# YzM1a0/MuDPT

Hardware: AMD Instinct MI355X
Metric: images/sec fwd+bwd ViT-B/16 MuDPT (higher is better)
Workload: dtype bf16; 1 GPU; MuDPT ViT-B/16 fwd+bwd+SGD, batch 256/GPU, 11 class prompts, n_ctx 4, depth 12, synthetic 224x224 N(0,1) images, random-init frozen CLIP (BASELINE configs[1]); global_batch=256, parallelism=dp1

## Files before the change

mudpt_amd/csrc/gemm.hip:

```cpp
#include <type_traits>

#include "kernels.h"

namespace mudpt {

using gptr_t = const __attribute__((address_space(1))) void*;
using lptr_t = __attribute__((address_space(3))) void*;

template <typename T, int BM, int BN, int WM, int WN, int EPI, int NS = 2, int BK = 64>
__global__ __launch_bounds__(WM* WN * 64) void gemm_nt_kernel(GemmArgs p) {
    using elem = typename T::elem;
    using vec8 = typename T::vec8;
    constexpr int NW = WM * WN;
    static_assert(BK == 64 || BK == 128, "K-tile");
    constexpr int ROWB = BK * 2;
    constexpr int RPI = 1024 / ROWB;
    constexpr int CPR = ROWB / 16;
    constexpr int TM = BM / WM / 16;
    constexpr int TN = BN / WN / 16;
    constexpr int IA = BM / RPI / NW;
    constexpr int IB = BN / RPI / NW;
    constexpr int STAGE_BYTES = (BM + BN) * ROWB;
    static_assert(BM % (RPI * NW) == 0 && BN % (RPI * NW) == 0, "tile rows must split over the waves");

    extern __shared__ __attribute__((aligned(16))) char smem[];

    const int tid = threadIdx.x;
    const int lane = tid & 63;
    const int wave = __builtin_amdgcn_readfirstlane(tid >> 6);
    const int wm = wave / WN, wn = wave % WN;

    const int ntn = (p.N + BN - 1) / BN;
    const int wg = (p.flags & 1) ? (int)blockIdx.x : xcd_remap(blockIdx.x, gridDim.x);
    const int m0 = (wg / ntn) * BM;
    const int n0 = (wg % ntn) * BN;

    const int kz = blockIdx.y, kspan = p.ksplit ? p.ksplit : p.K;
    const elem* __restrict__ A = (const elem*)p.A + (size_t)kz * kspan;
    const elem* __restrict__ Bw = (const elem*)p.B + (size_t)kz * kspan;

    const int srow = lane / CPR;
    const elem* asrc[IA];
    const elem* bsrc[IB];
#pragma unroll
    for (int i = 0; i < IA; ++i) {
        const int tr = (wave + NW * i) * RPI + srow;
        int r = m0 + tr;
        r = r < p.M ? r : p.M - 1;
        asrc[i] = A + (size_t)r * p.lda + ((lane % CPR) ^ (tr & (CPR - 1))) * 8;
    }
#pragma unroll
    for (int i = 0; i < IB; ++i) {
        const int tr = (wave + NW * i) * RPI + srow;
        int r = n0 + tr;
        r = r < p.N ? r : p.N - 1;
        bsrc[i] = Bw + (size_t)r * p.ldb + ((lane % CPR) ^ (tr & (CPR - 1))) * 8;
    }

    const int nt1 = kspan / BK;
    const bool f8 = p.lo_mode == LO_F8;
    const int nt = nt1 + (p.lo_mode == LO_NONE ? 0 : (f8 ? nt1 / 2 : nt1));
    const ptrdiff_t dA = p.A_lo ? (const char*)p.A_lo - (const char*)p.A : 0;
    const ptrdiff_t dB = f8 ? (const char*)p.B8 - (const char*)p.B : 0;
    auto stage = [&](int buf, int kt) {
        char* base = smem + buf * STAGE_BYTES;
        const bool second = kt >= nt1;
        const ptrdiff_t oa = second ? dA + (ptrdiff_t)(kt - nt1) * ROWB : (ptrdiff_t)kt * ROWB;
        const ptrdiff_t ob = second ? dB + (ptrdiff_t)(kt - nt1) * ROWB : (ptrdiff_t)kt * ROWB;
#pragma unroll
        for (int i = 0; i < IA; ++i)
            __builtin_amdgcn_global_load_lds((gptr_t)((const char*)asrc[i] + oa), (lptr_t)(base + (wave + NW * i) * 1024), 16, 0, 0);
#pragma unroll
        for (int i = 0; i < IB; ++i)
            __builtin_amdgcn_global_load_lds((gptr_t)((const char*)bsrc[i] + ob), (lptr_t)(base + BM * ROWB + (wave + NW * i) * 1024), 16, 0, 0);
    };

    f32x4 acc[TM][TN];
#pragma unroll
    for (int i = 0; i < TM; ++i)
#pragma unroll
        for (int j = 0; j < TN; ++j) acc[i][j] = f32x4{0.f, 0.f, 0.f, 0.f};

    const int frow = lane & 15;
    const int fq = lane >> 4;
    int aoff[TM], boff[TN];
#pragma unroll
    for (int i = 0; i < TM; ++i) aoff[i] = (wm * (BM / WM) + i * 16 + frow) * ROWB;
#pragma unroll
    for (int j = 0; j < TN; ++j) boff[j] = BM * ROWB + (wn * (BN / WN) + j * 16 + frow) * ROWB;
    const int sw = frow & (CPR - 1);

    static_assert(NS >= 2 && (NS & (NS - 1)) == 0, "ring depth must be a power of two");
#pragma unroll
    for (int st = 0; st < NS - 1; ++st)
        if (st < nt) stage(st, st);

    auto tile = [&](auto f8tag, int kt) {
        const int cur = kt & (NS - 1);
        if (kt + NS - 2 < nt) asm volatile("s_waitcnt vmcnt(%0)" ::"n"((NS - 2) * (IA + IB)) : "memory");
        else asm volatile("s_waitcnt vmcnt(0)" ::: "memory");
        __syncthreads();
        if (kt + NS - 1 < nt) stage((kt + NS - 1) & (NS - 1), kt + NS - 1);
        const char* base = smem + cur * STAGE_BYTES;
        if constexpr (decltype(f8tag)::value && BK == 64) {
            const int c = ((2 * fq) ^ sw) * 16;
            typedef __attribute__((ext_vector_type(4))) int i32x4;
            i32x8 b8[TN];
#pragma unroll
            for (int j = 0; j < TN; ++j)
                b8[j] = __builtin_shufflevector(*(const i32x4*)(base + boff[j] + c), *(const i32x4*)(base + boff[j] + (c ^ 16)), 0, 1, 2, 3, 4, 5, 6, 7);
#pragma unroll
            for (int i = 0; i < TM; ++i) {
                const i32x8 a8 = __builtin_shufflevector(*(const i32x4*)(base + aoff[i] + c), *(const i32x4*)(base + aoff[i] + (c ^ 16)), 0, 1, 2, 3, 4, 5, 6, 7);
#pragma unroll
                for (int j = 0; j < TN; ++j)
                    acc[i][j] = __builtin_amdgcn_mfma_scale_f32_16x16x128_f8f6f4(b8[j], a8, acc[i][j], 0, 0, 0, p.b8_scale, 0, LO8_SCALE_E8M0);
            }
        } else {
#pragma unroll
            for (int ks = 0; ks < BK / 32; ++ks) {
                const int c = ((ks * 4 + fq) ^ sw) * 16;
                vec8 af[TM], bf[TN];
#pragma unroll
                for (int i = 0; i < TM; ++i) af[i] = *(const vec8*)(base + aoff[i] + c);
#pragma unroll
                for (int j = 0; j < TN; ++j) bf[j] = *(const vec8*)(base + boff[j] + c);
#pragma unroll
                for (int i = 0; i < TM; ++i)
#pragma unroll
                    for (int j = 0; j < TN; ++j) acc[i][j] = T::mfma16(bf[j], af[i], acc[i][j]);
            }
        }
    };
    const int nt16 = f8 ? nt1 : nt;
    for (int kt = 0; kt < nt16; ++kt) tile(std::false_type{}, kt);
    for (int kt = nt16; kt < nt; ++kt) tile(std::true_type{}, kt);

#pragma unroll
    for (int i = 0; i < TM; ++i) {
        const int m = m0 + wm * (BM / WM) + i * 16 + frow;
        if (m >= p.M) continue;
        size_t orow = (size_t)m;
        const float* posrow = nullptr;
        if constexpr (EPI == EPI_PATCH) {
            const int b = m / p.patches, pp = m - b * p.patches;
            orow = (size_t)b * p.seq_len + 1 + pp;
            posrow = p.pos + (size_t)(1 + pp) * p.N;
        }
#pragma unroll
        for (int j = 0; j < TN; ++j) {
            const int n = n0 + wn * (BN / WN) + j * 16 + fq * 4;
            if (n >= p.N) continue;
            f32x4 v = acc[i][j];
            if (p.bias) {
                const f32x4 b4 = *(const f32x4*)(p.bias + n);
                v += b4;
            }
            if constexpr (EPI == EPI_STORE) {
                typename T::vec4 o = {round_to<elem>(v[0]), round_to<elem>(v[1]), round_to<elem>(v[2]), round_to<elem>(v[3])};
                *(typename T::vec4*)((elem*)p.out0 + orow * p.ldo0 + n) = o;
            } else if constexpr (EPI == EPI_GELU) {
                if (p.gelu_q8) {
                    *(uint32_t*)((char*)p.out0 + orow * p.ldo0 + n) = gelu_grad_q8x4(v[0], v[1], v[2], v[3]);
                } else {
                    typename T::vec4 u = {round_to<elem>(v[0]), round_to<elem>(v[1]), round_to<elem>(v[2]), round_to<elem>(v[3])};
                    *(typename T::vec4*)((elem*)p.out0 + orow * p.ldo0 + n) = u;
                }
                if (p.out1_lo) {
                    typename T::vec4 g, lo;
                    float rem[4];
#pragma unroll
                    for (int c = 0; c < 4; ++c) { elem hv; rem[c] = split_rem(quick_gelu(v[c]), hv); g[c] = hv; lo[c] = (elem)rem[c]; }
                    *(typename T::vec4*)((elem*)p.out1 + orow * p.ldo1 + n) = g;
                    if (p.out1_lo_mode == LO_F8) *(uint32_t*)((char*)p.out1_lo + orow * p.ldo1 * 2 + n) = pack_lo8(rem[0], rem[1], rem[2], rem[3]);
                    else *(typename T::vec4*)((elem*)p.out1_lo + orow * p.ldo1 + n) = lo;
                } else {
                    typename T::vec4 g = {round_to<elem>(quick_gelu(v[0])), round_to<elem>(quick_gelu(v[1])), round_to<elem>(quick_gelu(v[2])), round_to<elem>(quick_gelu(v[3]))};
                    *(typename T::vec4*)((elem*)p.out1 + orow * p.ldo1 + n) = g;
                }
            } else if constexpr (EPI == EPI_RESIDUAL) {
                const f32x4 r4 = *(const f32x4*)((const float*)p.aux + orow * p.ldaux + n);
                *(f32x4*)((float*)p.out0 + orow * p.ldo0 + n) = v + r4;
            } else if constexpr (EPI == EPI_GELU_BWD) {
                typename T::vec4 o;
                if (p.gelu_q8) {
                    const uint32_t w = *(const uint32_t*)((const char*)p.aux + orow * p.ldaux + n);
#pragma unroll
                    for (int c = 0; c < 4; ++c) o[c] = round_to<elem>(v[c] * gelu_grad_from_q8(w, c));
                } else {
                    const typename T::vec4 u = *(const typename T::vec4*)((const elem*)p.aux + orow * p.ldaux + n);
#pragma unroll
                    for (int c = 0; c < 4; ++c) o[c] = round_to<elem>(v[c] * quick_gelu_grad((float)u[c]));
                }
                *(typename T::vec4*)((elem*)p.out0 + orow * p.ldo0 + n) = o;
            } else if constexpr (EPI == EPI_PATCH) {
                const f32x4 q4 = *(const f32x4*)(posrow + n);
                *(f32x4*)((float*)p.out0 + orow * p.ldo0 + n) = v + q4;
            } else {
                *(f32x4*)((float*)p.out0 + (size_t)kz * p.split_stride + orow * p.ldo0 + n) = v;
            }
        }
    }
}

template <typename T, int BM, int BN, int WM, int WN, int EPI, int NS = 2, int BK = 64>
static int launch_cfg(const GemmArgs& a, hipStream_t s) {
    constexpr int lds = NS * (BM + BN) * BK * 2;
    constexpr auto kern = gemm_nt_kernel<T, BM, BN, WM, WN, EPI, NS, BK>;
    if (int e = lds_limit_once<kern>(current_device(), lds)) return e;
    const int ntm = (a.M + BM - 1) / BM, ntn = (a.N + BN - 1) / BN;
    hipLaunchKernelGGL(kern, dim3(ntm * ntn, a.ksplit ? a.K / a.ksplit : 1), dim3(WM * WN * 64), lds, s, a);
    HIP_TRY(hipGetLastError());
    return MUDPT_OK;
}

static inline bool small_tiles(const GemmArgs& a) {
    const size_t t64 = (size_t)((a.M + 63) / 64) * ((a.N + 63) / 64);
    return t64 <= 1280 || (t64 <= 2560 && a.K <= 512);
}

int device_cus(int dev) {
    static int ncu[64] = {};
    if (ncu[dev] <= 0) {
        const hipError_t e = hipDeviceGetAttribute(&ncu[dev], hipDeviceAttributeMultiprocessorCount, dev);
        if (e != hipSuccess) {
            set_error("%s:%d: hipDeviceGetAttribute(MultiprocessorCount, device %d) -> %s", __FILE__, __LINE__, dev, hipGetErrorString(e));
            return ncu[dev] = 0;
        }
    }
    return ncu[dev];
}
static int cus_or_256() {
    const int n = device_cus(current_device());
    return n > 0 ? n : 256;
}

static inline bool deep_k_tiles(const GemmArgs& a, int slices, int variant, int ncu) {
    const size_t t64 = (size_t)((a.M + 63) / 64) * ((a.N + 63) / 64);
    return (variant & 0xff) != 12 && a.lo_mode == LO_NONE && (a.K / slices) % 128 == 0 && t64 * slices <= (size_t)2 * ncu;
}

static GemmForm tile_form(const GemmArgs& a, int variant, int ncu) {
    if ((size_t)a.M * a.N >= (size_t)256 * 128 * 512) {
        switch (variant & 0xff) {
            case 2: return GEMM_T128x256;
            case 4: return GEMM_T256x128;
            default: return GEMM_T256x256;
        }
    }
    const size_t t128 = (size_t)((a.M + 127) / 128) * ((a.N + 127) / 128);
    const int v = variant & 0xff;
    if (((v == 0 && small_tiles(a)) || v == 10) && deep_k_tiles(a, 1, variant, ncu)) return GEMM_T64x64_K128;
    if (((v == 0 || v == 12) && small_tiles(a)) || v == 9 || v == 10) return GEMM_T64x64;
    if ((t128 <= 128 && v != 5) || v == 6) return GEMM_T128x64_RING4;
    return GEMM_T128x128;
}

template <typename T, int EPI>
static int launch_epi(GemmForm f, const GemmArgs& a, hipStream_t s) {
    switch (f) {
        case GEMM_T256x256: return launch_cfg<T, 256, 256, 2, 4, EPI>(a, s);
        case GEMM_T128x256: return launch_cfg<T, 128, 256, 2, 4, EPI>(a, s);
        case GEMM_T256x128: return launch_cfg<T, 256, 128, 4, 2, EPI>(a, s);
        case GEMM_T64x64_K128: return launch_cfg<T, 64, 64, 2, 2, EPI, 2, 128>(a, s);
        case GEMM_T64x64: return launch_cfg<T, 64, 64, 2, 2, EPI, 2>(a, s);
        case GEMM_T128x64_RING4: return launch_cfg<T, 128, 64, 2, 2, EPI, 4>(a, s);
        case GEMM_T128x128: return launch_cfg<T, 128, 128, 2, 2, EPI>(a, s);
        default: break;
    }
    set_error("gemm: form %d is not a simple tile", (int)f);
    return MUDPT_ERR_ARG;
}

template <typename T>
static int launch_t(int epi, GemmForm f, const GemmArgs& a, hipStream_t s) {
    switch (epi) {
        case EPI_STORE: return launch_epi<T, EPI_STORE>(f, a, s);
        case EPI_GELU: return launch_epi<T, EPI_GELU>(f, a, s);
        case EPI_RESIDUAL: return launch_epi<T, EPI_RESIDUAL>(f, a, s);
        case EPI_GELU_BWD: return launch_epi<T, EPI_GELU_BWD>(f, a, s);
        case EPI_PATCH: return launch_epi<T, EPI_PATCH>(f, a, s);
        case EPI_STORE_F32: return launch_epi<T, EPI_STORE_F32>(f, a, s);
    }
    set_error("gemm: unknown epilogue %d", epi);
    return MUDPT_ERR_ARG;
}

template <typename T, bool OUT_F32>
__global__ __launch_bounds__(256) void splitk_reduce_kernel(const float* __restrict__ part, int S, size_t stride, int M, int N, const float* __restrict__ bias,
                                                            void* __restrict__ out, int ldo) {
    const size_t i = (size_t)blockIdx.x * 256 + threadIdx.x, n4 = (size_t)N / 4;
    if (i >= (size_t)M * n4) return;
    const size_t m = i / n4, n = (i - m * n4) * 4;
    f32x4 v = *(const f32x4*)(part + m * N + n);
    for (int z = 1; z < S; ++z) v += *(const f32x4*)(part + (size_t)z * stride + m * N + n);
    if (bias) v += *(const f32x4*)(bias + n);
    if constexpr (OUT_F32) {
        *(f32x4*)((float*)out + m * ldo + n) = v;
    } else {
        using elem = typename T::elem;
        typename T::vec4 o = {round_to<elem>(v[0]), round_to<elem>(v[1]), round_to<elem>(v[2]), round_to<elem>(v[3])};
        *(typename T::vec4*)((elem*)out + m * ldo + n) = o;
    }
}

static int split_k_slices(int epi, const GemmArgs& a, const GemmOpts& o, int ncu, bool& deep) {
    deep = false;
    const int v = o.variant & 0xff;
    if (!(epi == EPI_STORE || epi == EPI_STORE_F32) || !o.scratch || (v != 0 && v != 12) || a.lo_mode != LO_NONE) return 1;
    const size_t tiles = (size_t)((a.M + 63) / 64) * ((a.N + 63) / 64);
    if (tiles * 2 > (size_t)ncu * 5 || a.K < 1536) return 1;
    int S = (int)((size_t)ncu * 2 / tiles);
    if (S > 4) S = 4;
    while (S > 1 && (a.K % (S * 128) != 0 || a.K / S < 512)) --S;
    if (S >= 3 && deep_k_tiles(a, S, o.variant, ncu) && (size_t)S * a.M * a.N <= o.scratch_elems) { deep = true; return S; }
    S = (int)((size_t)ncu * 5 / tiles);
    if (S > 4) S = 4;
    while (S > 1 && (a.K % (S * 64) != 0 || a.K / S < 512)) --S;
    if ((size_t)S * a.M * a.N > o.scratch_elems) return 1;
    return S;
}

bool gemm_uses_pp(int epi, const GemmArgs& a, int variant) {
    const bool pp_epi = epi == EPI_STORE || epi == EPI_GELU || epi == EPI_GELU_BWD || epi == EPI_STORE_F32;
    const int v = variant & 0xff;
    const size_t tiles = (size_t)((a.M + 255) / 256) * ((a.N + 255) / 256);
    return (v == 0 || v == 3 || v == 5 || v == 6 || v == 12) && pp_epi && tiles >= (v == 3 ? 256 : 128) && a.ldo0 % 8 == 0 && (epi != EPI_GELU || a.ldo1 % 8 == 0) &&
           (epi != EPI_GELU_BWD || a.ldaux % 8 == 0);
}

GemmPlan gemm_form(int epi, const GemmArgs& a, const GemmOpts& o, int ncu) {
    if (gemm_uses_pp(epi, a, o.variant)) return {GEMM_PP, 1};
    bool deep = false;
    if (const int S = split_k_slices(epi, a, o, ncu, deep); S > 1) return {deep ? GEMM_SPLITK_K128 : GEMM_SPLITK_K64, S};
    return {tile_form(a, o.variant, ncu), 1};
}

bool gemm_shape_ok(int epi, const GemmArgs& a) {
    if (epi < EPI_STORE || epi > EPI_STORE_F32) return false;
    if (!(a.M > 0 && a.N > 0 && a.K > 0) || a.K % 64 != 0 || a.N % 16 != 0) return false;
    if (!(a.ldo0 >= a.N && a.ldo0 % 4 == 0)) return false;
    if (epi == EPI_GELU && !(a.ldo1 >= a.N && a.ldo1 % 4 == 0)) return false;
    if ((epi == EPI_RESIDUAL || epi == EPI_GELU_BWD) && !(a.ldaux >= a.N && a.ldaux % 4 == 0)) return false;
    if (!(a.lo_mode == LO_NONE || a.lo_mode == LO_F16 || a.lo_mode == LO_F8)) return false;
    return a.lo_mode != LO_F8 || a.K % 128 == 0;
}

int launch_gemm(int dtype, int epi, const GemmArgs& a, hipStream_t s, const GemmOpts& o) {
    const int variant = o.variant;
    ARG_CHECK(a.A && a.B && a.out0, "gemm: null operand");
    ARG_CHECK(a.M > 0 && a.N > 0 && a.K > 0, "gemm: empty shape M=%d N=%d K=%d", a.M, a.N, a.K);
    ARG_CHECK(a.K % 64 == 0, "gemm: K=%d must be a multiple of 64", a.K);
    ARG_CHECK(a.N % 16 == 0, "gemm: N=%d must be a multiple of 16", a.N);
    ARG_CHECK(a.lda >= a.K && a.ldb >= a.K && a.lda % 8 == 0 && a.ldb % 8 == 0, "gemm: bad lda/ldb %d/%d", a.lda, a.ldb);
    ARG_CHECK(a.ldo0 >= a.N && a.ldo0 % 4 == 0, "gemm: bad ldo0 %d", a.ldo0);
    ARG_CHECK(((uintptr_t)a.A % 16 == 0) && ((uintptr_t)a.B % 16 == 0) && ((uintptr_t)a.out0 % 16 == 0), "gemm: operands must be 16-byte aligned");
    if (epi == EPI_GELU) ARG_CHECK(a.out1 && a.ldo1 >= a.N && a.ldo1 % 4 == 0, "gemm: gelu epilogue needs out1");
    ARG_CHECK(!a.out1_lo || a.out1_lo_mode == LO_F16 || a.out1_lo_mode == LO_F8, "gemm: bad out1_lo_mode %d", a.out1_lo_mode);
    ARG_CHECK(!a.gelu_q8 || ((epi == EPI_GELU && !a.out1_lo) || epi == EPI_GELU_BWD), "gemm: gelu_q8 belongs to the QuickGELU epilogues (1 without a split output, 3)");
    ARG_CHECK(a.lo_mode == LO_NONE || a.lo_mode == LO_F16 || a.lo_mode == LO_F8, "gemm: bad lo_mode %d", a.lo_mode);
    if (a.lo_mode != LO_NONE) ARG_CHECK(a.A_lo && (uintptr_t)a.A_lo % 16 == 0, "gemm: a split operand needs its low half (16-byte aligned)");
    if (a.lo_mode == LO_F8) {
        ARG_CHECK(dtype == DT_F16, "gemm: the e4m3 second pass exists for fp16 operands only");
        ARG_CHECK(a.B8 && (uintptr_t)a.B8 % 16 == 0 && a.K % 128 == 0, "gemm: the e4m3 second pass needs B8 and K %% 128 == 0 (K = %d)", a.K);
        ARG_CHECK(a.b8_scale > 0 && a.b8_scale < 255, "gemm: bad E8M0 weight scale %d", a.b8_scale);
    }
    if (epi == EPI_RESIDUAL || epi == EPI_GELU_BWD) ARG_CHECK(a.aux && a.ldaux >= a.N && a.ldaux % 4 == 0, "gemm: epilogue needs aux");
    if (epi == EPI_PATCH) ARG_CHECK(a.pos && a.patches > 0 && a.seq_len > a.patches && a.M % a.patches == 0, "gemm: bad patch epilogue args");
    GemmArgs b = a;
    if (variant & 0x100) b.flags |= 1;
    if (variant & 0x200) b.flags |= 2;
    b.flags |= ((variant >> 10) & 3) << 4;
    b.flags |= ((variant >> 12) & 0xff) << 8;
    const GemmPlan plan = gemm_form(epi, a, o, cus_or_256());
    if (plan.form == GEMM_PP) return launch_gemm_pp(dtype, epi, b, s, o);
    if (plan.slices > 1) {
        const int S = plan.slices;
        const bool deep = plan.form == GEMM_SPLITK_K128;
        GemmArgs q = b;
        q.bias = nullptr; q.out0 = o.scratch; q.ldo0 = a.N; q.ksplit = a.K / S; q.split_stride = (size_t)a.M * a.N;
        if (dtype == DT_BF16) { if (int rc = deep ? launch_cfg<BF16, 64, 64, 2, 2, EPI_STORE_F32, 2, 128>(q, s) : launch_cfg<BF16, 64, 64, 2, 2, EPI_STORE_F32, 2>(q, s)) return rc; }
        else if (dtype == DT_F16) { if (int rc = deep ? launch_cfg<F16, 64, 64, 2, 2, EPI_STORE_F32, 2, 128>(q, s) : launch_cfg<F16, 64, 64, 2, 2, EPI_STORE_F32, 2>(q, s)) return rc; }
        else { set_error("gemm: unknown dtype %d", dtype); return MUDPT_ERR_ARG; }
        const unsigned grid = (unsigned)(((size_t)a.M * (a.N / 4) + 255) / 256);
        if (epi == EPI_STORE_F32) hipLaunchKernelGGL((splitk_reduce_kernel<BF16, true>), dim3(grid), dim3(256), 0, s, o.scratch, S, q.split_stride, a.M, a.N, a.bias, a.out0, a.ldo0);
        else if (dtype == DT_BF16) hipLaunchKernelGGL((splitk_reduce_kernel<BF16, false>), dim3(grid), dim3(256), 0, s, o.scratch, S, q.split_stride, a.M, a.N, a.bias, a.out0, a.ldo0);
        else hipLaunchKernelGGL((splitk_reduce_kernel<F16, false>), dim3(grid), dim3(256), 0, s, o.scratch, S, q.split_stride, a.M, a.N, a.bias, a.out0, a.ldo0);
        HIP_TRY(hipGetLastError());
        return MUDPT_OK;
    }
    if (dtype == DT_BF16) return launch_t<BF16>(epi, plan.form, b, s);
    if (dtype == DT_F16) return launch_t<F16>(epi, plan.form, b, s);
    set_error("gemm: unknown dtype %d", dtype);
    return MUDPT_ERR_ARG;
}

}
```

mudpt_amd/csrc/gemm_pp.hip:

```cpp
#include <hip/hip_ext.h>

#include <type_traits>

#include "kernels.h"

namespace mudpt {

using lptr_t = __attribute__((address_space(3))) void*;

#define VMCNT(n) asm volatile("s_waitcnt vmcnt(" #n ")" ::: "memory")
typedef __attribute__((ext_vector_type(4))) unsigned int u32x4;

template <int N>
__device__ inline void vmcnt() {
    static_assert(N >= 0 && N <= 63, "vmcnt immediate is 6 bits");
    asm volatile("s_waitcnt vmcnt(%0)" ::"n"(N) : "memory");
}

constexpr int EPI_GELU_SPLIT = 100;
constexpr int EPI_GELU_SPLIT8 = 101;
constexpr int EPI_GELU_Q8 = 102;
constexpr int EPI_GELU_BWD_Q8 = 103;

template <typename T, int EPI, bool F8 = false, int ST = 0, int LD = 0, int ABL = 0>
__global__ __launch_bounds__(512) void gemm_pp_kernel(GemmArgs p, int ntn, int ntiles, int rem_half) {
    using elem = typename T::elem;
    using vec8 = typename T::vec8;
    constexpr int STAGE = 65536, BOFF = 32768;
    extern __shared__ __attribute__((aligned(16))) char smem[];

    const int tid = threadIdx.x, lane = tid & 63;
    const int w = __builtin_amdgcn_readfirstlane(tid >> 6);
    const int wr = w >> 2, wc = w & 3;
    const int frow = lane & 15, fq = lane >> 4;

    const int nkt1 = p.K >> 6;
    const int nkt = nkt1 + (p.lo_mode == LO_NONE ? 0 : (F8 ? nkt1 >> 1 : nkt1));
    const int G = gridDim.x;
    const int my_full = rem_half ? ntiles / G : (ntiles - (int)blockIdx.x + G - 1) / G;
    const bool has_half = rem_half && (int)blockIdx.x < 2 * rem_half;
    const int total = (my_full + (has_half ? 1 : 0)) * nkt;

    const auto rsA = __builtin_amdgcn_make_buffer_rsrc(const_cast<void*>(p.A), 0, (int)((size_t)p.M * p.lda * 2 < 0xffffffffull ? (size_t)p.M * p.lda * 2 : 0xffffffffull), 0x00020000);
    const auto rsB = __builtin_amdgcn_make_buffer_rsrc(const_cast<void*>(p.B), 0, (int)((size_t)p.N * p.ldb * 2 < 0xffffffffull ? (size_t)p.N * p.ldb * 2 : 0xffffffffull), 0x00020000);
    const auto rsA2 = __builtin_amdgcn_make_buffer_rsrc(const_cast<void*>(p.A_lo ? p.A_lo : p.A), 0, (int)((size_t)p.M * p.lda * 2 < 0xffffffffull ? (size_t)p.M * p.lda * 2 : 0xffffffffull), 0x00020000);
    const auto rsB2 = __builtin_amdgcn_make_buffer_rsrc(const_cast<void*>(F8 ? p.B8 : p.B), 0, (int)((size_t)p.N * p.ldb * 2 < 0xffffffffull ? (size_t)p.N * p.ldb * 2 : 0xffffffffull), 0x00020000);

    static_assert(EPI == EPI_STORE || EPI == EPI_GELU || EPI == EPI_GELU_SPLIT || EPI == EPI_GELU_SPLIT8 || EPI == EPI_GELU_BWD || EPI == EPI_STORE_F32 ||
                  EPI == EPI_GELU_Q8 || EPI == EPI_GELU_BWD_Q8, "epilogue not built for gemm_pp");
    constexpr bool GELU = (EPI == EPI_GELU || EPI == EPI_GELU_SPLIT || EPI == EPI_GELU_SPLIT8 || EPI == EPI_GELU_Q8);
    constexpr int OOB = (int)0x80000000;
    constexpr bool OUT_F32 = (EPI == EPI_STORE_F32);
    constexpr bool NAT = OUT_F32;
    constexpr int NST = (EPI == EPI_STORE || EPI == EPI_GELU_BWD || EPI == EPI_GELU_BWD_Q8) ? 16 : (EPI == EPI_GELU_SPLIT ? 48 : (EPI == EPI_GELU_SPLIT8 ? 40 : (EPI == EPI_GELU_Q8 ? 24 : 32)));
    const auto rsOut0 = __builtin_amdgcn_make_buffer_rsrc(p.out0, 0, p.M * p.ldo0 * (OUT_F32 ? 4 : (EPI == EPI_GELU_Q8 ? 1 : 2)), 0x00020000);
    const auto rsOut1 = __builtin_amdgcn_make_buffer_rsrc(p.out1, 0, GELU ? p.M * p.ldo1 * 2 : 0, 0x00020000);
    const auto rsOut1Lo = __builtin_amdgcn_make_buffer_rsrc(p.out1_lo, 0, (EPI == EPI_GELU_SPLIT || EPI == EPI_GELU_SPLIT8) ? p.M * p.ldo1 * 2 : 0, 0x00020000);
    const auto rsAux = __builtin_amdgcn_make_buffer_rsrc(const_cast<void*>(p.aux), 0, EPI == EPI_GELU_BWD ? p.M * p.ldaux * 2 : (EPI == EPI_GELU_BWD_Q8 ? p.M * p.ldaux : 0), 0x00020000);
    const auto rsBias = __builtin_amdgcn_make_buffer_rsrc(const_cast<float*>(p.bias), 0, p.bias ? p.N * 4 : 0, 0x00020000);
    bool epi_pending = false;

    int grp[4][2];
#pragma unroll
    for (int q = 0; q < 2; ++q) {
        const int k = 2 * w + q;
        grp[0][q] = k < 8 ? k : k + 8;
        grp[3][q] = k < 8 ? k + 8 : k + 16;
        grp[1][q] = NAT ? (k >> 2) * 8 + (k & 3) : 2 * k;
        grp[2][q] = NAT ? (k >> 2) * 8 + (k & 3) + 4 : 2 * k + 1;
    }
    const int srow = lane >> 3, sslot = lane & 7;
    int lane_off[4][2];
#pragma unroll
    for (int u = 0; u < 4; ++u)
#pragma unroll
        for (int q = 0; q < 2; ++q) {
            const bool isA = (u == 0 || u == 3);
            const int row = grp[u][q] * 8 + srow;
            const int f = (isA || NAT) ? (row & 7) : ((row & 3) | (((row >> 4) & 1) << 2));
            lane_off[u][q] = (row * (isA ? p.lda : p.ldb) + ((sslot ^ f) << 3)) * 2;
        }

    const int gn_knob = (p.flags >> 8) & 0xff;
    const int GN = gn_knob > 0 ? gn_knob : (ntn >= 12 ? 6 : (ntn >= 6 && ntn % 3 == 0 ? 3 : ntn));
    const int ntm = ntiles / ntn;
    auto tile_mn = [&](int tile, int& tm, int& tn) {
        const int tpg = ntm * GN, full = ntn / GN, ng = tile / tpg;
        if (ng < full) {
            const int rem = tile - ng * tpg;
            tm = rem / GN;
            tn = ng * GN + (rem - tm * GN);
        } else {
            const int wl = ntn - full * GN, rem = tile - full * tpg;
            tm = rem / wl;
            tn = full * GN + (rem - tm * wl);
        }
    };
    auto item_tile = [&](int it, int& tm, int& tn, int& h) {
        if (it < my_full) {
            tile_mn(xcd_remap((int)blockIdx.x + it * G, ntiles), tm, tn);
            h = 0;
        } else {
            h = (int)blockIdx.x >= rem_half ? 1 : 0;
            tile_mn(xcd_remap(my_full * G + (int)blockIdx.x - h * rem_half, ntiles), tm, tn);
        }
    };
    int n_kt = 0, n_it = 0, n_baseA = 0, n_baseB = 0, n_soff = 0;
    bool n_second = false;
    bool n_half = false;
    auto set_next_item = [&](int it) {
        int tm, tn, h;
        item_tile(it, tm, tn, h);
        n_half = it >= my_full;
        n_baseA = (tm * 256 + (n_half ? h * 128 - (w >= 4 ? 64 : 0) : 0)) * p.lda * 2;
        n_baseB = tn * 256 * p.ldb * 2;
    };
    auto advance_next = [&]() {
        n_soff += 128;
        if (++n_kt == nkt) {
            n_kt = 0; n_soff = 0; n_second = false;
            if ((++n_it) * nkt < total) set_next_item(n_it);
        } else if (n_kt == nkt1) {
            n_soff = 0; n_second = true;
        }
    };
    auto issue = [&](int u, int stage) {
        if constexpr (ABL & 2) return;
        const bool isA = (u == 0 || u == 3);
        const int base = isA ? n_baseA : n_baseB;
        char* dst = smem + stage * STAGE + (isA ? 0 : BOFF);
#pragma unroll
        for (int q = 0; q < 2; ++q)
            __builtin_amdgcn_raw_ptr_buffer_load_lds(isA ? (n_second ? rsA2 : rsA) : (n_second ? rsB2 : rsB), (lptr_t)(dst + grp[u][q] * 1024), 16, lane_off[u][q] + base, n_soff, 0, 0);
    };

    const int sw = frow & 7;
    const int c0 = (fq ^ sw) << 4;
    const int c8 = ((2 * fq) ^ sw) << 4;
    int ca = c0, cb = c0 ^ 64;
    const int a_base = (wr * 128 + frow) * 128;
    const int b_base = BOFF + (NAT ? wc * 64 + frow : wc * 64 + (frow >> 2) * 16 + (frow & 3)) * 128;
    constexpr int BJ = NAT ? 2048 : 512;

    f32x4 acc[8][4];
#pragma unroll
    for (int i = 0; i < 8; ++i)
#pragma unroll
        for (int j = 0; j < 4; ++j) acc[i][j] = f32x4{0.f, 0.f, 0.f, 0.f};

    if (total > 0) {
        set_next_item(0);
        issue(0, 0); issue(1, 0); issue(2, 0);
        if (!n_half) issue(3, 0);
        advance_next();
    }
    VMCNT(0);
    __builtin_amdgcn_s_barrier();
    if (wr == 1) __builtin_amdgcn_s_barrier();

    typedef __attribute__((ext_vector_type(4))) int i32x4;
    i32x8 af[4], bf[4];
    if constexpr (ABL & 1) {
#pragma unroll
        for (int i = 0; i < 4; ++i) { af[i] = i32x8{lane, 1, 2, 3, 4, 5, 6, 7} * 0x3c003c00; bf[i] = i32x8{7, 6, 5, 4, 3, 2, 1, lane} * 0x3c003c00; }
    }
    auto half = [](const i32x8& v, int ks) -> vec8 {
        return __builtin_bit_cast(vec8, ks ? __builtin_shufflevector(v, v, 4, 5, 6, 7) : __builtin_shufflevector(v, v, 0, 1, 2, 3));
    };
    int c_it = 0;

    auto mfma_quadrant = [&](auto f8tag, int i0, int j0) {
        __builtin_amdgcn_sched_barrier(0);
        __builtin_amdgcn_s_setprio(1);
        if constexpr (decltype(f8tag)::value) {
#pragma unroll
            for (int i = 0; i < 4; ++i)
#pragma unroll
                for (int j = 0; j < 2; ++j)
                    acc[i0 + i][j0 + j] = __builtin_amdgcn_mfma_scale_f32_16x16x128_f8f6f4(bf[j0 + j], af[i], acc[i0 + i][j0 + j], 0, 0, 0, p.b8_scale, 0, LO8_SCALE_E8M0);
        } else {
#pragma unroll
            for (int ks = 0; ks < 2; ++ks)
#pragma unroll
                for (int i = 0; i < 4; ++i)
#pragma unroll
                    for (int j = 0; j < 2; ++j) acc[i0 + i][j0 + j] = T::mfma16(half(bf[j0 + j], ks), half(af[i], ks), acc[i0 + i][j0 + j]);
        }
        __builtin_amdgcn_s_setprio(0);
        __builtin_amdgcn_sched_barrier(0);
    };
    auto read_a = [&](const char* st, int i0) {
        if constexpr (ABL & 1) return;
#pragma unroll
        for (int i = 0; i < 4; ++i)
            af[i] = __builtin_shufflevector(*(const i32x4*)(st + a_base + (i0 + i) * 2048 + ca), *(const i32x4*)(st + a_base + (i0 + i) * 2048 + cb), 0, 1, 2, 3, 4, 5, 6, 7);
    };
    auto read_b = [&](const char* st, int j0) {
        if constexpr (ABL & 1) return;
#pragma unroll
        for (int j = j0; j < j0 + 2; ++j)
            bf[j] = __builtin_shufflevector(*(const i32x4*)(st + b_base + j * BJ + ca), *(const i32x4*)(st + b_base + j * BJ + cb), 0, 1, 2, 3, 4, 5, 6, 7);
    };
    auto epilogue = [&]() {
            int tm, tn, h;
            const bool c_half = c_it >= my_full;
            item_tile(c_it++, tm, tn, h);
            const int ni = c_half ? 4 : 8;
            const int n = tn * 256 + wc * 64 + (NAT ? fq * 4 : fq * 16);
            f32x4 bias4[4];
#pragma unroll
            for (int j = 0; j < 4; ++j)
                bias4[j] = p.bias ? __builtin_bit_cast(f32x4, __builtin_amdgcn_raw_buffer_load_b128(rsBias, (n + (NAT ? 16 : 4) * j) * 4, 0, 0)) : f32x4{0.f, 0.f, 0.f, 0.f};
            const int m_base = tm * 256 + (c_half ? h * 128 + wr * 64 : wr * 128) + frow;
            auto row_off = [&](int i, int ld, int esz, int col) { return (col < p.N ? (m_base * ld + col) * esz : OOB) + i * (16 * ld * esz); };
#pragma unroll
            for (int i = 0; i < 8; ++i)
#pragma unroll
                for (int j = 0; j < 4; ++j) acc[i][j] += bias4[j];
            if constexpr (EPI == EPI_GELU_BWD) {
                vec8 u[8][2];
#pragma unroll
                for (int i = 0; i < 8; ++i) {
                    const int off = i < ni ? row_off(i, p.ldaux, 2, n) : OOB;
                    u[i][0] = __builtin_bit_cast(vec8, __builtin_amdgcn_raw_buffer_load_b128(rsAux, off, 0, LD));
                    u[i][1] = __builtin_bit_cast(vec8, __builtin_amdgcn_raw_buffer_load_b128(rsAux, off, 16, LD));
                }
#pragma unroll
                for (int i = 0; i < 8; ++i)
#pragma unroll
                    for (int j = 0; j < 4; ++j)
#pragma unroll
                        for (int c = 0; c < 4; ++c) acc[i][j][c] *= quick_gelu_grad((float)u[i][j >> 1][4 * (j & 1) + c]);
            }
            if constexpr (EPI == EPI_GELU_BWD_Q8) {
                u32x4 q[8];
#pragma unroll
                for (int i = 0; i < 8; ++i) q[i] = __builtin_amdgcn_raw_buffer_load_b128(rsAux, i < ni ? row_off(i, p.ldaux, 1, n) : OOB, 0, LD);
#pragma unroll
                for (int i = 0; i < 8; ++i)
#pragma unroll
                    for (int j = 0; j < 4; ++j)
#pragma unroll
                        for (int c = 0; c < 4; ++c) acc[i][j][c] *= gelu_grad_from_q8(q[i][j], c);
            }
            __builtin_amdgcn_sched_barrier(0);
#pragma unroll
            for (int i = 0; i < 8; ++i) {
                if (i < ni) {
                if constexpr (OUT_F32) {
#pragma unroll
                    for (int j = 0; j < 4; ++j) __builtin_amdgcn_raw_buffer_store_b128(__builtin_bit_cast(u32x4, acc[i][j]), rsOut0, row_off(i, p.ldo0, 4, n + 16 * j), 0, ST);
                } else {
                    vec8 o0, o1;
                    if constexpr (EPI == EPI_GELU_Q8) {
                        u32x4 q;
#pragma unroll
                        for (int j = 0; j < 4; ++j) q[j] = gelu_grad_q8x4(acc[i][j][0], acc[i][j][1], acc[i][j][2], acc[i][j][3]);
                        __builtin_amdgcn_raw_buffer_store_b128(q, rsOut0, row_off(i, p.ldo0, 1, n), 0, ST);
                    } else {
#pragma unroll
                        for (int c = 0; c < 4; ++c) {
                            o0[c] = round_to<elem>(acc[i][0][c]); o0[4 + c] = round_to<elem>(acc[i][1][c]);
                            o1[c] = round_to<elem>(acc[i][2][c]); o1[4 + c] = round_to<elem>(acc[i][3][c]);
                        }
                        const int off = row_off(i, p.ldo0, 2, n);
                        __builtin_amdgcn_raw_buffer_store_b128(__builtin_bit_cast(u32x4, o0), rsOut0, off, 0, ST);
                        __builtin_amdgcn_raw_buffer_store_b128(__builtin_bit_cast(u32x4, o1), rsOut0, off, 16, ST);
                    }
                    if constexpr (EPI == EPI_GELU || EPI == EPI_GELU_Q8) {
#pragma unroll
                        for (int c = 0; c < 4; ++c) {
                            o0[c] = round_to<elem>(quick_gelu(acc[i][0][c])); o0[4 + c] = round_to<elem>(quick_gelu(acc[i][1][c]));
                            o1[c] = round_to<elem>(quick_gelu(acc[i][2][c])); o1[4 + c] = round_to<elem>(quick_gelu(acc[i][3][c]));
                        }
                        const int off1 = row_off(i, p.ldo1, 2, n);
                        __builtin_amdgcn_raw_buffer_store_b128(__builtin_bit_cast(u32x4, o0), rsOut1, off1, 0, ST);
                        __builtin_amdgcn_raw_buffer_store_b128(__builtin_bit_cast(u32x4, o1), rsOut1, off1, 16, ST);
                    }
                    if constexpr (EPI == EPI_GELU_SPLIT8) {
                        u32x4 l8;
                        float rem[4];
#pragma unroll
                        for (int j = 0; j < 4; ++j) {
#pragma unroll
                            for (int c = 0; c < 4; ++c) {
                                elem hv;
                                rem[c] = split_rem(quick_gelu(acc[i][j][c]), hv);
                                if (j < 2) o0[4 * j + c] = hv; else o1[4 * (j - 2) + c] = hv;
                            }
                            l8[j] = pack_lo8(rem[0], rem[1], rem[2], rem[3]);
                        }
                        const int off1 = row_off(i, p.ldo1, 2, n);
                        __builtin_amdgcn_raw_buffer_store_b128(__builtin_bit_cast(u32x4, o0), rsOut1, off1, 0, ST);
                        __builtin_amdgcn_raw_buffer_store_b128(__builtin_bit_cast(u32x4, o1), rsOut1, off1, 16, ST);
                        __builtin_amdgcn_raw_buffer_store_b128(l8, rsOut1Lo, (n < p.N ? m_base * p.ldo1 * 2 + n : OOB) + i * (32 * p.ldo1), 0, ST);
                    }
                    if constexpr (EPI == EPI_GELU_SPLIT) {
                        vec8 l0, l1;
#pragma unroll
                        for (int c = 0; c < 4; ++c) {
                            elem hv, lv;
                            split_hi_lo(quick_gelu(acc[i][0][c]), hv, lv); o0[c] = hv; l0[c] = lv;
                            split_hi_lo(quick_gelu(acc[i][1][c]), hv, lv); o0[4 + c] = hv; l0[4 + c] = lv;
                            split_hi_lo(quick_gelu(acc[i][2][c]), hv, lv); o1[c] = hv; l1[c] = lv;
                            split_hi_lo(quick_gelu(acc[i][3][c]), hv, lv); o1[4 + c] = hv; l1[4 + c] = lv;
                        }
                        const int off1 = row_off(i, p.ldo1, 2, n);
                        __builtin_amdgcn_raw_buffer_store_b128(__builtin_bit_cast(u32x4, o0), rsOut1, off1, 0, ST);
                        __builtin_amdgcn_raw_buffer_store_b128(__builtin_bit_cast(u32x4, o1), rsOut1, off1, 16, ST);
                        __builtin_amdgcn_raw_buffer_store_b128(__builtin_bit_cast(u32x4, l0), rsOut1Lo, off1, 0, ST);
                        __builtin_amdgcn_raw_buffer_store_b128(__builtin_bit_cast(u32x4, l1), rsOut1Lo, off1, 16, ST);
                    }
                }
                }
#pragma unroll
                for (int j = 0; j < 4; ++j) acc[i][j] = f32x4{0.f, 0.f, 0.f, 0.f};
            }
            epi_pending = true;
    };

    int s = 0;
    auto full_step = [&](auto f8tag) {
        constexpr bool F8S = decltype(f8tag)::value;
        const int cur = s & 1;
        const char* st = smem + cur * STAGE;
        const bool nxt = s + 1 < total;
        ca = F8S ? c8 : c0;
        cb = F8S ? (c8 ^ 16) : (c0 ^ 64);
        read_a(st, 0);
        read_b(st, 0);
        if (nxt) {
            issue(0, cur ^ 1);
            if (epi_pending) vmcnt<NST + 4>(); else vmcnt<4>();
        } else {
            if (epi_pending) vmcnt<NST + 2>(); else vmcnt<2>();
        }
        __builtin_amdgcn_s_barrier();
        mfma_quadrant(f8tag, 0, 0);
        __builtin_amdgcn_s_barrier();
        read_b(st, 2);
        if (nxt) {
            issue(1, cur ^ 1);
            if (epi_pending) vmcnt<NST + 4>(); else vmcnt<4>();
        } else {
            if (epi_pending) vmcnt<NST>(); else vmcnt<0>();
        }
        epi_pending = false;
        __builtin_amdgcn_s_barrier();
        mfma_quadrant(f8tag, 0, 2);
        __builtin_amdgcn_s_barrier();
        read_a(st, 4);
        if (nxt) issue(2, cur ^ 1);
        __builtin_amdgcn_s_barrier();
        mfma_quadrant(f8tag, 4, 2);
        __builtin_amdgcn_s_barrier();
        if (nxt) {
            if (!n_half) { issue(3, cur ^ 1); advance_next(); VMCNT(4); } else { advance_next(); VMCNT(2); }
        }
        __builtin_amdgcn_s_barrier();
        mfma_quadrant(f8tag, 4, 0);
        __builtin_amdgcn_s_barrier();
        ++s;
    };
    auto half_step = [&](auto f8tag) {
        constexpr bool F8S = decltype(f8tag)::value;
        const int cur = s & 1;
        const char* st = smem + cur * STAGE;
        const bool nxt = s + 1 < total;
        ca = F8S ? c8 : c0;
        cb = F8S ? (c8 ^ 16) : (c0 ^ 64);
        read_a(st, 0);
        read_b(st, 0);
        if (nxt) {
            issue(0, cur ^ 1);
            issue(1, cur ^ 1);
            if (epi_pending) vmcnt<NST + 4>(); else vmcnt<4>();
        } else {
            if (epi_pending) vmcnt<NST>(); else vmcnt<0>();
        }
        __builtin_amdgcn_s_barrier();
        mfma_quadrant(f8tag, 0, 0);
        __builtin_amdgcn_s_barrier();
        read_b(st, 2);
        if (nxt) { issue(2, cur ^ 1); advance_next(); VMCNT(2); }
        epi_pending = false;
        __builtin_amdgcn_s_barrier();
        mfma_quadrant(f8tag, 0, 2);
        __builtin_amdgcn_s_barrier();
        ++s;
    };
    const int nkt2 = nkt - nkt1;
    for (int it = 0; it < my_full; ++it) {
        if constexpr (F8) {
            for (int k = 0; k < nkt1; ++k) full_step(std::false_type{});
            for (int k = 0; k < nkt2; ++k) full_step(std::true_type{});
        } else {
            for (int k = 0; k < nkt; ++k) full_step(std::false_type{});
        }
        epilogue();
    }
    if (has_half) {
        if constexpr (F8) {
            for (int k = 0; k < nkt1; ++k) half_step(std::false_type{});
            for (int k = 0; k < nkt2; ++k) half_step(std::true_type{});
        } else {
            for (int k = 0; k < nkt; ++k) half_step(std::false_type{});
        }
        epilogue();
    }
    if (wr == 0) __builtin_amdgcn_s_barrier();
}

template <typename T, int EPI, bool F8 = false, int ST = 0, int LD = 0, int ABL = 0>
static int launch_pp(const GemmArgs& a, hipStream_t s, const GemmOpts& o) {
    constexpr int lds = 2 * 65536;
    constexpr auto kern = gemm_pp_kernel<T, EPI, F8, ST, LD, ABL>;
    const int dev = current_device(), ncu = device_cus(dev);
    if (ncu <= 0) return MUDPT_ERR_HIP;
    if (int e = lds_limit_once<kern>(dev, lds)) return e;
    const int ntm = (a.M + 255) / 256, ntn = (a.N + 255) / 256, ntiles = ntm * ntn;
    int grid = ntiles < ncu ? (2 * ntiles <= ncu ? 2 * ntiles : ntiles) : ncu;
    if (a.flags & 2) grid = ntiles < ncu ? ntiles : ncu;
    const int rem = ntiles % grid, rem_half = (rem > 0 && 2 * rem <= grid && !(a.flags & 2)) ? rem : 0;
    if (o.ev_start && o.ev_stop) {
        hipExtLaunchKernelGGL(kern, dim3(grid), dim3(512), lds, s, o.ev_start, o.ev_stop, 0, a, ntn, ntiles, rem_half);
    } else {
        hipLaunchKernelGGL(kern, dim3(grid), dim3(512), lds, s, a, ntn, ntiles, rem_half);
    }
    HIP_TRY(hipGetLastError());
    return MUDPT_OK;
}

template <typename T>
static int launch_pp_t(int epi, const GemmArgs& a, hipStream_t s, const GemmOpts& o) {
    if constexpr (T::id == DT_F16) {
        if (a.lo_mode == LO_F8) {
            switch (epi) {
                case EPI_STORE: return launch_pp<T, EPI_STORE, true>(a, s, o);
                case EPI_GELU:
                    if (!a.out1_lo) return launch_pp<T, EPI_GELU, true>(a, s, o);
                    return a.out1_lo_mode == LO_F8 ? launch_pp<T, EPI_GELU_SPLIT8, true>(a, s, o) : launch_pp<T, EPI_GELU_SPLIT, true>(a, s, o);
                case EPI_STORE_F32: return launch_pp<T, EPI_STORE_F32, true>(a, s, o);
            }
            set_error("gemm_pp: epilogue %d is not built with the e4m3 second pass", epi);
            return MUDPT_ERR_ARG;
        }
    }
    if constexpr (T::id == DT_BF16) {
        if (epi == EPI_STORE && (a.flags & 0x30)) {
            switch ((a.flags >> 4) & 3) {
                case 1: return launch_pp<T, EPI_STORE, false, 0, 0, 1>(a, s, o);
                case 2: return launch_pp<T, EPI_STORE, false, 0, 0, 2>(a, s, o);
                default: return launch_pp<T, EPI_STORE, false, 0, 0, 3>(a, s, o);
            }
        }
    }
    switch (epi) {
        case EPI_STORE: return launch_pp<T, EPI_STORE>(a, s, o);
        case EPI_GELU:
            if (!a.out1_lo) return a.gelu_q8 ? launch_pp<T, EPI_GELU_Q8>(a, s, o) : launch_pp<T, EPI_GELU>(a, s, o);
            return a.out1_lo_mode == LO_F8 ? launch_pp<T, EPI_GELU_SPLIT8>(a, s, o) : launch_pp<T, EPI_GELU_SPLIT>(a, s, o);
        case EPI_GELU_BWD: return a.gelu_q8 ? launch_pp<T, EPI_GELU_BWD_Q8>(a, s, o) : launch_pp<T, EPI_GELU_BWD>(a, s, o);
        case EPI_STORE_F32: return launch_pp<T, EPI_STORE_F32>(a, s, o);
    }
    set_error("gemm_pp: epilogue %d is not built for the ping-pong kernel", epi);
    return MUDPT_ERR_ARG;
}

int launch_gemm_pp(int dtype, int epi, const GemmArgs& a, hipStream_t s, const GemmOpts& o) {
    ARG_CHECK((size_t)a.M * a.lda * 2 < 0xffffffffull && (size_t)a.N * a.ldb * 2 < 0xffffffffull, "gemm_pp: operand larger than 4 GiB");
    ARG_CHECK(a.lda % 8 == 0 && a.ldb % 8 == 0 && a.ldo0 % 8 == 0, "gemm_pp: strides must be multiples of 8");
    ARG_CHECK(!a.out1_lo || (uintptr_t)a.out1_lo % 16 == 0, "gemm_pp: out1_lo must be 16-byte aligned");
    ARG_CHECK(!a.gelu_q8 || (a.lo_mode == LO_NONE && a.ldo0 % 16 == 0 && a.ldaux % 16 == 0), "gemm_pp: gelu_q8 needs 16-byte row strides and no split operand");
    ARG_CHECK((size_t)a.M * a.ldo0 * (epi == EPI_STORE_F32 ? 4 : 2) < 0x7fffffffull && (size_t)a.M * (size_t)(a.ldo1 > a.ldaux ? a.ldo1 : a.ldaux) * 2 < 0x7fffffffull, "gemm_pp: output larger than 2 GiB");
    if (dtype == DT_BF16) return launch_pp_t<BF16>(epi, a, s, o);
    if (dtype == DT_F16) return launch_pp_t<F16>(epi, a, s, o);
    set_error("gemm: unknown dtype %d", dtype);
    return MUDPT_ERR_ARG;
}

}
```

Measured before the change: 10870 images/s.

## Remap ping-pong GEMM B-fragment layout for dense epilogue stores, add cache-policy variants

Changes how B rows are assigned to LDS groups and which output columns each lane owns, so dense epilogues (store, GELU, GELU-bwd, q8) write two split column chunks per row instead of one contiguous 32-byte span. The q8 paths move from 128-bit to 64-bit loads and stores, and the stride check is relaxed to match. It also adds a variant bit field that selects nontemporal store or load cache policies per output for bf16 kernels. This affects the default store pattern of every dense ping-pong GEMM and could change coalescing either way.

Result: no change. 10840 images/s (-0.2%).

```diff
diff --git a/mudpt_amd/csrc/gemm.hip b/mudpt_amd/csrc/gemm.hip
--- a/mudpt_amd/csrc/gemm.hip
+++ b/mudpt_amd/csrc/gemm.hip
@@ -372,6 +372,7 @@
     if (variant & 0x200) b.flags |= 2;
     b.flags |= ((variant >> 10) & 3) << 4;
     b.flags |= ((variant >> 12) & 0xff) << 8;
+    b.flags |= ((variant >> 20) & 3) << 16;
     const GemmPlan plan = gemm_form(epi, a, o, cus_or_256());
     if (plan.form == GEMM_PP) return launch_gemm_pp(dtype, epi, b, s, o);
     if (plan.slices > 1) {
diff --git a/mudpt_amd/csrc/gemm_pp.hip b/mudpt_amd/csrc/gemm_pp.hip
--- a/mudpt_amd/csrc/gemm_pp.hip
+++ b/mudpt_amd/csrc/gemm_pp.hip
@@ -10,6 +10,7 @@
 
 #define VMCNT(n) asm volatile("s_waitcnt vmcnt(" #n ")" ::: "memory")
 typedef __attribute__((ext_vector_type(4))) unsigned int u32x4;
+typedef __attribute__((ext_vector_type(2))) unsigned int u32x2;
 
 template <int N>
 __device__ inline void vmcnt() {
@@ -22,8 +23,9 @@
 constexpr int EPI_GELU_Q8 = 102;
 constexpr int EPI_GELU_BWD_Q8 = 103;
 
-template <typename T, int EPI, bool F8 = false, int ST = 0, int LD = 0, int ABL = 0>
+template <typename T, int EPI, bool F8 = false, int ST = 0, int LD = 0, int ABL = 0, int ST1 = ST>
 __global__ __launch_bounds__(512) void gemm_pp_kernel(GemmArgs p, int ntn, int ntiles, int rem_half) {
+    constexpr int ST0 = ST;
     using elem = typename T::elem;
     using vec8 = typename T::vec8;
     constexpr int STAGE = 65536, BOFF = 32768;
@@ -52,7 +54,8 @@
     constexpr int OOB = (int)0x80000000;
     constexpr bool OUT_F32 = (EPI == EPI_STORE_F32);
     constexpr bool NAT = OUT_F32;
-    constexpr int NST = (EPI == EPI_STORE || EPI == EPI_GELU_BWD || EPI == EPI_GELU_BWD_Q8) ? 16 : (EPI == EPI_GELU_SPLIT ? 48 : (EPI == EPI_GELU_SPLIT8 ? 40 : (EPI == EPI_GELU_Q8 ? 24 : 32)));
+    constexpr bool DENSE = !NAT && EPI != EPI_GELU_SPLIT && EPI != EPI_GELU_SPLIT8;
+    constexpr int NST = (EPI == EPI_STORE || EPI == EPI_GELU_BWD || EPI == EPI_GELU_BWD_Q8) ? 16 : (EPI == EPI_GELU_SPLIT ? 48 : (EPI == EPI_GELU_SPLIT8 ? 40 : 32));
     const auto rsOut0 = __builtin_amdgcn_make_buffer_rsrc(p.out0, 0, p.M * p.ldo0 * (OUT_F32 ? 4 : (EPI == EPI_GELU_Q8 ? 1 : 2)), 0x00020000);
     const auto rsOut1 = __builtin_amdgcn_make_buffer_rsrc(p.out1, 0, GELU ? p.M * p.ldo1 * 2 : 0, 0x00020000);
     const auto rsOut1Lo = __builtin_amdgcn_make_buffer_rsrc(p.out1_lo, 0, (EPI == EPI_GELU_SPLIT || EPI == EPI_GELU_SPLIT8) ? p.M * p.ldo1 * 2 : 0, 0x00020000);
@@ -66,8 +69,8 @@
         const int k = 2 * w + q;
         grp[0][q] = k < 8 ? k : k + 8;
         grp[3][q] = k < 8 ? k + 8 : k + 16;
-        grp[1][q] = NAT ? (k >> 2) * 8 + (k & 3) : 2 * k;
-        grp[2][q] = NAT ? (k >> 2) * 8 + (k & 3) + 4 : 2 * k + 1;
+        grp[1][q] = (NAT || DENSE) ? (k >> 2) * 8 + (k & 3) : 2 * k;
+        grp[2][q] = (NAT || DENSE) ? (k >> 2) * 8 + (k & 3) + 4 : 2 * k + 1;
     }
     const int srow = lane >> 3, sslot = lane & 7;
     int lane_off[4][2];
@@ -77,7 +80,7 @@
         for (int q = 0; q < 2; ++q) {
             const bool isA = (u == 0 || u == 3);
             const int row = grp[u][q] * 8 + srow;
-            const int f = (isA || NAT) ? (row & 7) : ((row & 3) | (((row >> 4) & 1) << 2));
+            const int f = (isA || NAT) ? (row & 7) : ((row & 3) | (((row >> (DENSE ? 3 : 4)) & 1) << 2));
             lane_off[u][q] = (row * (isA ? p.lda : p.ldb) + ((sslot ^ f) << 3)) * 2;
         }
 
@@ -139,8 +142,8 @@
     const int c8 = ((2 * fq) ^ sw) << 4;
     int ca = c0, cb = c0 ^ 64;
     const int a_base = (wr * 128 + frow) * 128;
-    const int b_base = BOFF + (NAT ? wc * 64 + frow : wc * 64 + (frow >> 2) * 16 + (frow & 3)) * 128;
-    constexpr int BJ = NAT ? 2048 : 512;
+    const int b_base = BOFF + (NAT ? wc * 64 + frow : wc * 64 + (frow >> 2) * (DENSE ? 8 : 16) + (frow & 3)) * 128;
+    auto bj = [](int j) { return NAT ? j * 2048 : (DENSE ? (j & 1) * 512 + (j >> 1) * 4096 : j * 512); };
 
     f32x4 acc[8][4];
 #pragma unroll
@@ -199,18 +202,20 @@
         if constexpr (ABL & 1) return;
 #pragma unroll
         for (int j = j0; j < j0 + 2; ++j)
-            bf[j] = __builtin_shufflevector(*(const i32x4*)(st + b_base + j * BJ + ca), *(const i32x4*)(st + b_base + j * BJ + cb), 0, 1, 2, 3, 4, 5, 6, 7);
+            bf[j] = __builtin_shufflevector(*(const i32x4*)(st + b_base + bj(j) + ca), *(const i32x4*)(st + b_base + bj(j) + cb), 0, 1, 2, 3, 4, 5, 6, 7);
     };
     auto epilogue = [&]() {
             int tm, tn, h;
             const bool c_half = c_it >= my_full;
             item_tile(c_it++, tm, tn, h);
             const int ni = c_half ? 4 : 8;
-            const int n = tn * 256 + wc * 64 + (NAT ? fq * 4 : fq * 16);
+            const int n = tn * 256 + wc * 64 + (NAT ? fq * 4 : (DENSE ? fq * 8 : fq * 16));
+            constexpr int P1 = DENSE ? 32 : 8;
+            auto colj = [](int j) { return NAT ? 16 * j : (DENSE ? 4 * (j & 1) + 32 * (j >> 1) : 4 * j); };
             f32x4 bias4[4];
 #pragma unroll
             for (int j = 0; j < 4; ++j)
-                bias4[j] = p.bias ? __builtin_bit_cast(f32x4, __builtin_amdgcn_raw_buffer_load_b128(rsBias, (n + (NAT ? 16 : 4) * j) * 4, 0, 0)) : f32x4{0.f, 0.f, 0.f, 0.f};
+                bias4[j] = p.bias ? __builtin_bit_cast(f32x4, __builtin_amdgcn_raw_buffer_load_b128(rsBias, (n + colj(j)) * 4, 0, 0)) : f32x4{0.f, 0.f, 0.f, 0.f};
             const int m_base = tm * 256 + (c_half ? h * 128 + wr * 64 : wr * 128) + frow;
             auto row_off = [&](int i, int ld, int esz, int col) { return (col < p.N ? (m_base * ld + col) * esz : OOB) + i * (16 * ld * esz); };
 #pragma unroll
@@ -221,9 +226,8 @@
                 vec8 u[8][2];
 #pragma unroll
                 for (int i = 0; i < 8; ++i) {
-                    const int off = i < ni ? row_off(i, p.ldaux, 2, n) : OOB;
-                    u[i][0] = __builtin_bit_cast(vec8, __builtin_amdgcn_raw_buffer_load_b128(rsAux, off, 0, LD));
-                    u[i][1] = __builtin_bit_cast(vec8, __builtin_amdgcn_raw_buffer_load_b128(rsAux, off, 16, LD));
+                    u[i][0] = __builtin_bit_cast(vec8, __builtin_amdgcn_raw_buffer_load_b128(rsAux, i < ni ? row_off(i, p.ldaux, 2, n) : OOB, 0, LD));
+                    u[i][1] = __builtin_bit_cast(vec8, __builtin_amdgcn_raw_buffer_load_b128(rsAux, i < ni ? row_off(i, p.ldaux, 2, n + P1) : OOB, 0, LD));
                 }
 #pragma unroll
                 for (int i = 0; i < 8; ++i)
@@ -233,15 +237,18 @@
                         for (int c = 0; c < 4; ++c) acc[i][j][c] *= quick_gelu_grad((float)u[i][j >> 1][4 * (j & 1) + c]);
             }
             if constexpr (EPI == EPI_GELU_BWD_Q8) {
-                u32x4 q[8];
-#pragma unroll
-                for (int i = 0; i < 8; ++i) q[i] = __builtin_amdgcn_raw_buffer_load_b128(rsAux, i < ni ? row_off(i, p.ldaux, 1, n) : OOB, 0, LD);
+                u32x2 q[8][2];
+#pragma unroll
+                for (int i = 0; i < 8; ++i) {
+                    q[i][0] = __builtin_amdgcn_raw_buffer_load_b64(rsAux, i < ni ? row_off(i, p.ldaux, 1, n) : OOB, 0, LD);
+                    q[i][1] = __builtin_amdgcn_raw_buffer_load_b64(rsAux, i < ni ? row_off(i, p.ldaux, 1, n + P1) : OOB, 0, LD);
+                }
 #pragma unroll
                 for (int i = 0; i < 8; ++i)
 #pragma unroll
                     for (int j = 0; j < 4; ++j)
 #pragma unroll
-                        for (int c = 0; c < 4; ++c) acc[i][j][c] *= gelu_grad_from_q8(q[i][j], c);
+                        for (int c = 0; c < 4; ++c) acc[i][j][c] *= gelu_grad_from_q8(q[i][j >> 1][j & 1], c);
             }
             __builtin_amdgcn_sched_barrier(0);
 #pragma unroll
@@ -253,19 +260,19 @@
                 } else {
                     vec8 o0, o1;
                     if constexpr (EPI == EPI_GELU_Q8) {
-                        u32x4 q;
-#pragma unroll
-                        for (int j = 0; j < 4; ++j) q[j] = gelu_grad_q8x4(acc[i][j][0], acc[i][j][1], acc[i][j][2], acc[i][j][3]);
-                        __builtin_amdgcn_raw_buffer_store_b128(q, rsOut0, row_off(i, p.ldo0, 1, n), 0, ST);
+                        u32x2 q[2];
+#pragma unroll
+                        for (int j = 0; j < 4; ++j) q[j >> 1][j & 1] = gelu_grad_q8x4(acc[i][j][0], acc[i][j][1], acc[i][j][2], acc[i][j][3]);
+                        __builtin_amdgcn_raw_buffer_store_b64(q[0], rsOut0, row_off(i, p.ldo0, 1, n), 0, ST0);
+                        __builtin_amdgcn_raw_buffer_store_b64(q[1], rsOut0, row_off(i, p.ldo0, 1, n + P1), 0, ST0);
                     } else {
 #pragma unroll
                         for (int c = 0; c < 4; ++c) {
                             o0[c] = round_to<elem>(acc[i][0][c]); o0[4 + c] = round_to<elem>(acc[i][1][c]);
                             o1[c] = round_to<elem>(acc[i][2][c]); o1[4 + c] = round_to<elem>(acc[i][3][c]);
                         }
-                        const int off = row_off(i, p.ldo0, 2, n);
-                        __builtin_amdgcn_raw_buffer_store_b128(__builtin_bit_cast(u32x4, o0), rsOut0, off, 0, ST);
-                        __builtin_amdgcn_raw_buffer_store_b128(__builtin_bit_cast(u32x4, o1), rsOut0, off, 16, ST);
+                        __builtin_amdgcn_raw_buffer_store_b128(__builtin_bit_cast(u32x4, o0), rsOut0, row_off(i, p.ldo0, 2, n), 0, ST0);
+                        __builtin_amdgcn_raw_buffer_store_b128(__builtin_bit_cast(u32x4, o1), rsOut0, row_off(i, p.ldo0, 2, n + P1), 0, ST0);
                     }
                     if constexpr (EPI == EPI_GELU || EPI == EPI_GELU_Q8) {
 #pragma unroll
@@ -273,9 +280,8 @@
                             o0[c] = round_to<elem>(quick_gelu(acc[i][0][c])); o0[4 + c] = round_to<elem>(quick_gelu(acc[i][1][c]));
                             o1[c] = round_to<elem>(quick_gelu(acc[i][2][c])); o1[4 + c] = round_to<elem>(quick_gelu(acc[i][3][c]));
                         }
-                        const int off1 = row_off(i, p.ldo1, 2, n);
-                        __builtin_amdgcn_raw_buffer_store_b128(__builtin_bit_cast(u32x4, o0), rsOut1, off1, 0, ST);
-                        __builtin_amdgcn_raw_buffer_store_b128(__builtin_bit_cast(u32x4, o1), rsOut1, off1, 16, ST);
+                        __builtin_amdgcn_raw_buffer_store_b128(__builtin_bit_cast(u32x4, o0), rsOut1, row_off(i, p.ldo1, 2, n), 0, ST1);
+                        __builtin_amdgcn_raw_buffer_store_b128(__builtin_bit_cast(u32x4, o1), rsOut1, row_off(i, p.ldo1, 2, n + P1), 0, ST1);
                     }
                     if constexpr (EPI == EPI_GELU_SPLIT8) {
                         u32x4 l8;
@@ -411,10 +417,10 @@
     if (wr == 0) __builtin_amdgcn_s_barrier();
 }
 
-template <typename T, int EPI, bool F8 = false, int ST = 0, int LD = 0, int ABL = 0>
+template <typename T, int EPI, bool F8 = false, int ST = 0, int LD = 0, int ABL = 0, int ST1 = ST>
 static int launch_pp(const GemmArgs& a, hipStream_t s, const GemmOpts& o) {
     constexpr int lds = 2 * 65536;
-    constexpr auto kern = gemm_pp_kernel<T, EPI, F8, ST, LD, ABL>;
+    constexpr auto kern = gemm_pp_kernel<T, EPI, F8, ST, LD, ABL, ST1>;
     const int dev = current_device(), ncu = device_cus(dev);
     if (ncu <= 0) return MUDPT_ERR_HIP;
     if (int e = lds_limit_once<kern>(dev, lds)) return e;
@@ -455,6 +461,18 @@
             }
         }
     }
+    if constexpr (T::id == DT_BF16) {
+        constexpr int NT = 2;
+        const int pol = (a.flags >> 16) & 3;
+        if (pol == 1) {
+            if (epi == EPI_STORE) return launch_pp<T, EPI_STORE, false, NT>(a, s, o);
+            if (epi == EPI_GELU && !a.out1_lo && a.gelu_q8) return launch_pp<T, EPI_GELU_Q8, false, NT>(a, s, o);
+            if (epi == EPI_GELU_BWD && a.gelu_q8) return launch_pp<T, EPI_GELU_BWD_Q8, false, NT>(a, s, o);
+        } else if (pol == 2) {
+            if (epi == EPI_GELU && !a.out1_lo && a.gelu_q8) return launch_pp<T, EPI_GELU_Q8, false, NT, 0, 0, 0>(a, s, o);
+            if (epi == EPI_GELU_BWD && a.gelu_q8) return launch_pp<T, EPI_GELU_BWD_Q8, false, 0, NT>(a, s, o);
+        }
+    }
     switch (epi) {
         case EPI_STORE: return launch_pp<T, EPI_STORE>(a, s, o);
         case EPI_GELU:
@@ -471,7 +489,7 @@
     ARG_CHECK((size_t)a.M * a.lda * 2 < 0xffffffffull && (size_t)a.N * a.ldb * 2 < 0xffffffffull, "gemm_pp: operand larger than 4 GiB");
     ARG_CHECK(a.lda % 8 == 0 && a.ldb % 8 == 0 && a.ldo0 % 8 == 0, "gemm_pp: strides must be multiples of 8");
     ARG_CHECK(!a.out1_lo || (uintptr_t)a.out1_lo % 16 == 0, "gemm_pp: out1_lo must be 16-byte aligned");
-    ARG_CHECK(!a.gelu_q8 || (a.lo_mode == LO_NONE && a.ldo0 % 16 == 0 && a.ldaux % 16 == 0), "gemm_pp: gelu_q8 needs 16-byte row strides and no split operand");
+    ARG_CHECK(!a.gelu_q8 || (a.lo_mode == LO_NONE && a.ldo0 % 8 == 0 && a.ldaux % 8 == 0), "gemm_pp: gelu_q8 needs 8-byte row strides and no split operand");
     ARG_CHECK((size_t)a.M * a.ldo0 * (epi == EPI_STORE_F32 ? 4 : 2) < 0x7fffffffull && (size_t)a.M * (size_t)(a.ldo1 > a.ldaux ? a.ldo1 : a.ldaux) * 2 < 0x7fffffffull, "gemm_pp: output larger than 2 GiB");
     if (dtype == DT_BF16) return launch_pp_t<BF16>(epi, a, s, o);
     if (dtype == DT_F16) return launch_pp_t<F16>(epi, a, s, o);
```
